# jingjing12110/X-GGM

Measured on AMD Instinct MI355X. Metric: train samples/sec (36-obj VQA batch); one step = plain + GGM pass, each fwd+bwd+clip+BertAdam, higher is better.
Workload: dtype bf16; 1 GPU; 1xMI355X bf16: VQA-CP-v2-shaped synthetic batch=32/GPU, 36 objects x 2048, 20 tokens, A=2274, LXMERT 9/5/5 + GCNx2, full fwd+bwd+clip+BertAdam x2 passes (plain pass first, KL x 8), dropout on, delta=5 branch mix; global_batch=32, parallelism=dp1, order=vqa, world_size=1, zero1=False, hip_graph=True

## Files before the change

### include/xggm.h

```cpp
#ifndef XGGM_H
#define XGGM_H

#include <stddef.h>
#include <stdint.h>

#ifdef __cplusplus
extern "C" {
#endif

typedef struct ihipStream_t* xggm_stream_t;

#define XGGM_VERSION 100

#define XGGM_ACT_NONE 0
#define XGGM_ACT_GELU 1
#define XGGM_ACT_SIGMOID 2
#define XGGM_ACT_TANH 3
#define XGGM_ACT_GELU_GRAD 4

#define XGGM_AGG_PLAIN 0
#define XGGM_AGG_TRANSPOSE 1
#define XGGM_AGG_SYMMETRIZE 2

int xggm_version(void);
// ... 18 lines not shown
    int64_t a_bs, b_bs, c_bs;
    const float* bias;
    const void* residual;
    void* preact;
    const void* aux;
    float* colsum;
    int act, c_f32, accumulate;
    float alpha;
    float* sqsum;
    const float* scale_a;
    const float* scale_b;
    void* c8;
    const float* c8_qscale;
    float* c8_amax;
    int amax_slots;
} xggm_gemm_problem;
int xggm_gemm_grouped_f32(const xggm_gemm_problem* probs, int n, int tile, xggm_stream_t stream);
int xggm_gemm_grouped_bf16(const xggm_gemm_problem* probs, int n, int tile, xggm_stream_t stream);
int xggm_gemm_fp8e4m3(const void* A, const void* B, void* C, int M, int N, int K, int64_t a_rs, int64_t b_ns, int64_t ldc,
                      const float* scale_a, const float* scale_b, const float* bias, const void* residual, void* preact,
                      int act, int c_f32, xggm_stream_t stream);
int xggm_gemm_grouped_fp8e4m3(const xggm_gemm_problem* probs, int n, int tile, xggm_stream_t stream);
int xggm_fp8_scale_update(float* amax, float* hist, float* qscale, float* dscale, int64_t* pos, int n, int hist_len,
                          float margin, int shrink, int bump, int amax_slots, xggm_stream_t stream);
int xggm_quantize_fp8e4m3_f32(const void* x, void* y, int64_t n, const float* qscale, float* amax, xggm_stream_t stream);
int xggm_quantize_fp8e4m3_bf16(const void* x, void* y, int64_t n, const float* qscale, float* amax, xggm_stream_t stream);
int xggm_gemm_set_group_tile(int v);
int xggm_gemm_set_generic(int on);
int xggm_gemm_set_tile(int variant);
int xggm_colsum_f32(const void* x, float* out, int M, int N, int64_t ld, float* ws, size_t ws_bytes,
                    xggm_stream_t stream);
// ... 482 lines not shown
```

### x-ggm_amd/csrc/gemm.hip

```cpp
#include "common.h"
#include "xggm.h"

namespace {

typedef __attribute__((ext_vector_type(8))) short short8_t;
typedef __attribute__((ext_vector_type(4))) float float4_t;

struct GemmArgs {
    const void* A = nullptr;
    const void* B = nullptr;
    void* C = nullptr;
    int M = 0, N = 0, K = 0;
    int64_t a_rs = 0, a_ks = 0, b_ns = 0, b_ks = 0, ldc = 0;
    int64_t a_bs = 0, b_bs = 0, c_bs = 0;
    const float* bias = nullptr;
    const void* residual = nullptr;
    void* preact = nullptr;
    const void* aux = nullptr;
    float* colsum = nullptr;
    float* sqsum = nullptr;
    unsigned char* c8 = nullptr;
    const float* c8_qscale = nullptr;
    float* c8_amax = nullptr;
    int amax_slots = 1;
    const float* scale_a = nullptr;
    const float* scale_b = nullptr;
    int act = 0;
    int c_f32 = 0;
    int accumulate = 0;
    float alpha = 1.f;
    int a_mode = 0, b_mode = 0;
    int a_tail = 0, b_tail = 0;
    int a_rows = 0, b_rows = 0;
    int xcd_swizzle = 1;
    int batch = 1;
    int use_glds = 1;
    struct TileMap {
        int gx, gy, gxy;
        int xr, xc, rh, rw;
// ... 433 lines not shown
                    {
                        const float4 a = *reinterpret_cast<const float4*>(sp);
                        const float4 c4 = *reinterpret_cast<const float4*>(sp + 4);
                        v[0] = a.x; v[1] = a.y; v[2] = a.z; v[3] = a.w; v[4] = c4.x; v[5] = c4.y; v[6] = c4.z; v[7] = c4.w;
                    }
#pragma unroll
                    for (int e = 0; e < 8; ++e) v[e] = g.alpha * v[e] + bias[e];
                    if (pre) {
                        short8_t pv;
#pragma unroll
                        for (int e = 0; e < 8; ++e) {
                            const bf16 t = __float2bfloat16(v[e]);
                            pv[e] = __builtin_bit_cast(short, t);
                            v[e] = __bfloat162float(t);
                        }
                        *reinterpret_cast<short8_t*>(pre + idx[b]) = pv;
                    }
                    if (g.act == XGGM_ACT_GELU) {
#pragma unroll
                        for (int e = 0; e < 8; ++e) v[e] = gelu_f(v[e]);
                    } else if (g.act == XGGM_ACT_GELU_GRAD) {
#pragma unroll
                        for (int e = 0; e < 8; ++e)
                            v[e] *= gelu_grad_f(__bfloat162float(__builtin_bit_cast(bf16, (short)raux[b][e])));
                    } else if (g.act != XGGM_ACT_NONE) {
#pragma unroll 1
                        for (int e = 0; e < 8; ++e) v[e] = act_apply<bf16>(g.act, v[e], 0.f);
                    }
                    if (res) {
#pragma unroll
                        for (int e = 0; e < 8; ++e) v[e] += __bfloat162float(__builtin_bit_cast(bf16, (short)rres[b][e]));
                    }
                    if (g.colsum) {
                        *reinterpret_cast<float4*>(sp) = make_float4(v[0], v[1], v[2], v[3]);
                        *reinterpret_cast<float4*>(sp + 4) = make_float4(v[4], v[5], v[6], v[7]);
                    }
                    if (g.c8) {
#pragma unroll
                        for (int e = 0; e < 8; ++e) amax8 = fmaxf(amax8, fabsf(v[e]));
                        *reinterpret_cast<int2*>(g.c8 + idx[b]) =
                            make_int2(pack4_e4m3(v[0], v[1], v[2], v[3], q8), pack4_e4m3(v[4], v[5], v[6], v[7], q8));
                    }
                    if (g.c_f32) {
                        float* c = reinterpret_cast<float*>(g.C) + idx[b];
                        float4 o0 = make_float4(v[0], v[1], v[2], v[3]), o1 = make_float4(v[4], v[5], v[6], v[7]);
                        if (g.accumulate) {
                            o0.x += p0[b].x; o0.y += p0[b].y; o0.z += p0[b].z; o0.w += p0[b].w;
                            o1.x += p1[b].x; o1.y += p1[b].y; o1.z += p1[b].z; o1.w += p1[b].w;
                        }
                        if (g.sqsum)
                            sq_add(h * HALF + lr0 + (it0 + b) * RPI, (o0.x * o0.x + o0.y * o0.y) + (o0.z * o0.z + o0.w * o0.w) +
                                                                         (o1.x * o1.x + o1.y * o1.y) + (o1.z * o1.z + o1.w * o1.w));
                        typedef float __attribute__((ext_vector_type(4))) f4;
                        __builtin_nontemporal_store((f4){o0.x, o0.y, o0.z, o0.w}, reinterpret_cast<f4*>(c));
                        __builtin_nontemporal_store((f4){o1.x, o1.y, o1.z, o1.w}, reinterpret_cast<f4*>(c + 4));
                    } else {
                        if (g.accumulate) {
#pragma unroll
                            for (int e = 0; e < 8; ++e) v[e] += __bfloat162float(__builtin_bit_cast(bf16, (short)rprev[b][e]));
                        }
                        short8_t ov;
#pragma unroll
                        for (int e = 0; e < 8; ++e) ov[e] = __builtin_bit_cast(short, __float2bfloat16(v[e]));
                        *reinterpret_cast<short8_t*>(reinterpret_cast<bf16*>(g.C) + idx[b]) = ov;
                    }
                }
            }
        } else {
#pragma unroll 1
            for (int it = 0; it < ITER; ++it) {
                const int lr = lr0 + it * RPI, row = m0 + h * HALF + lr;
                if (row >= g.M || !col_ok) continue;
                const int nval = min(8, g.N - col);
                const int64_t idx = coff + (int64_t)row * g.ldc + col;
#pragma unroll 1
                for (int e = 0; e < nval; ++e) {
                    float x = g.alpha * stage[lr * LDS_LD + lc + e] + (g.bias ? g.bias[col + e] : 0.f);
                    if (pre) {
                        pre[idx + e] = __float2bfloat16(x);
// ... 95 lines not shown
#pragma unroll
    for (int j = 0; j < TN; ++j)
        bias[j] = (g.bias && col0 + j * 16 < g.N) ? *reinterpret_cast<const float4_t*>(g.bias + col0 + j * 16)
                                                  : (float4_t){0.f, 0.f, 0.f, 0.f};
    const Q8 qs(KIND == 1 && g.c8 ? g.c8_qscale : nullptr);
    const float q8 = qs.q, alpha = g.alpha;
    float amax8 = 0.f, sq = 0.f;
#ifdef XGGM_STAMP
    if (g.ablate & 0x10000) asm volatile("s_waitcnt vmcnt(0)" ::: "memory");
#endif
    TRACE(g, 1);
    const int off0 = row0 * g.ldc + col0;
    float* cf = reinterpret_cast<float*>(g.C) + coff;
    bf16* cb = reinterpret_cast<bf16*>(g.C) + coff;
    bf16* pre = reinterpret_cast<bf16*>(g.preact) + coff;
#pragma unroll
    for (int i = 0; i < TM; ++i) {
        if (i == 1) STAMP(g, 3);
        TRACE(g, 2 + i);
        if (row0 + i * 16 >= g.M) continue;
#pragma unroll
        for (int j = 0; j < TN; ++j) {
            if (col0 + j * 16 >= g.N) continue;
            const int off = off0 + i * 16 * g.ldc + j * 16;
            float4_t v = alpha * acc[i][j] + bias[j];
            if (KIND == 1) {
                short4v pv;
#pragma unroll
                for (int e = 0; e < 4; ++e) {
                    const bf16 t = __float2bfloat16(v[e]);
                    pv[e] = __builtin_bit_cast(short, t);
                    v[e] = gelu_f(__bfloat162float(t));
                }
                *reinterpret_cast<short4v*>(pre + off) = pv;
                if (g.c8) {
                    amax8 = fmaxf(fmaxf(amax8, fmaxf(fabsf(v[0]), fabsf(v[1]))), fmaxf(fabsf(v[2]), fabsf(v[3])));
                    *reinterpret_cast<int*>(g.c8 + coff + off) = pack4_e4m3(v[0], v[1], v[2], v[3], q8);
                }
            }
            if (KIND == 0 && g.c_f32) {
                sq += (v[0] * v[0] + v[1] * v[1]) + (v[2] * v[2] + v[3] * v[3]);
                __builtin_nontemporal_store(v, reinterpret_cast<float4_t*>(cf + off));
            } else {
                short4v ov;
#pragma unroll
                for (int e = 0; e < 4; ++e) ov[e] = __builtin_bit_cast(short, __float2bfloat16(v[e]));
                if (!ABLATE(g, 4) || ov[0] == 12345) *reinterpret_cast<short4v*>(cb + off) = ov;
            }
        }
    }
    if (KIND == 1 && g.c8 && g.c8_amax) {
        const float wv = wave_max(amax8);
        if (lane == 0) stage[wid] = wv;
        lds_barrier();
        if (tid == 0) {
            float bm = stage[0];
#pragma unroll
            for (int w = 1; w < W; ++w) bm = fmaxf(bm, stage[w]);
            if (bm > qs.thr) amax_record(g.c8_amax, g.amax_slots, (int)(blockIdx.x + blockIdx.y * gridDim.x), bm);
        }
    }
    if (KIND == 0 && g.sqsum) {
// ... 789 lines not shown
            *rows = (R + VEC - 1) / VEC * VEC;
            return 2;
        }
    }
    return 0;
}

GemmArgs from_problem(const xggm_gemm_problem& p, const GemmHooks& h) {
    GemmArgs g;
    g.A = p.A; g.B = p.B; g.C = p.C; g.M = p.M; g.N = p.N; g.K = p.K;
    g.a_rs = p.a_rs; g.a_ks = p.a_ks; g.b_ns = p.b_ns; g.b_ks = p.b_ks; g.ldc = p.ldc;
    g.a_bs = p.a_bs; g.b_bs = p.b_bs; g.c_bs = p.c_bs;
    g.bias = p.bias; g.residual = p.residual; g.preact = p.preact; g.aux = p.aux; g.colsum = p.colsum; g.sqsum = p.sqsum;
    g.c8 = reinterpret_cast<unsigned char*>(p.c8); g.c8_qscale = p.c8_qscale; g.c8_amax = p.c8_amax;
    g.amax_slots = p.amax_slots > 1 ? p.amax_slots : 1;
    g.scale_a = p.scale_a; g.scale_b = p.scale_b;
    g.act = p.act; g.c_f32 = p.c_f32; g.accumulate = p.accumulate; g.alpha = p.alpha;
    g.xcd_swizzle = h.xcd_swizzle; g.batch = p.batch; g.use_glds = h.glds; SET_STAMP(g);
    return g;
}

template <typename T> int launch(GemmArgs g, int batch, const GemmHooks& h, hipStream_t stream) {
    XGGM_REQUIRE(g.M > 0 && g.N > 0 && g.K > 0 && batch > 0, "xggm_gemm: empty problem M=%d N=%d K=%d batch=%d", g.M, g.N,
                 g.K, batch);
    XGGM_REQUIRE(g.A && g.B && g.C, "xggm_gemm: null operand");
    XGGM_REQUIRE(g.act >= 0 && g.act <= XGGM_ACT_GELU_GRAD, "xggm_gemm: bad activation %d", g.act);
    XGGM_REQUIRE(g.act != XGGM_ACT_GELU_GRAD || g.aux, "xggm_gemm: GELU_GRAD needs aux");
    XGGM_REQUIRE(g.ldc >= g.N, "xggm_gemm: ldc %lld < N %d", (long long)g.ldc, g.N);
    XGGM_REQUIRE(!g.sqsum || g.c_f32, "xggm_gemm: sqsum is defined for fp32 outputs");
    g.a_mode = pick_mode<T>(g.A, g.a_rs, g.a_ks, g.a_bs, g.M, g.K, &g.a_tail, &g.a_rows);
// ... 109 lines not shown
                nkmax = std::max(nkmax, nk);
            }
            const float r = std::max(1.0, tiles / 256.0);
            const float est = std::max(tm.a + tm.b * r + tm.s * (float)(work / 256.0), tm.f + tm.k * nkmax);
            if (v == 0 || est < best) {
                best = est;
                v = c + 1;
            }
        }
    }
    return v;
}

inline bool group_tile_ok(int tile) { return (tile >= 0 && tile <= 4) || (tile >= 7 && tile <= 9); }

template <typename T> int grouped(const xggm_gemm_problem* probs, int n, int tile, const GemmHooks h, hipStream_t stream) {
    XGGM_REQUIRE(probs && n > 0, "xggm_gemm_grouped: no problems");
    XGGM_REQUIRE(group_tile_ok(tile), "xggm_gemm_grouped: tile %d (0: the library chooses; 1-4, 7-9: see xggm.h)", tile);
    const int pin = tile ? tile : h.group_tile;
    bool fast = sizeof(T) == 2 && !h.force_generic && n <= MAX_GROUP;
    GroupArgs ga;
    ga.nprob = n;
    for (int i = 0; i < n && fast; ++i) {
        GemmArgs g = from_problem(probs[i], h);
        if (!(g.M > 0 && g.N > 0 && g.K > 0 && g.batch > 0 && g.A && g.B && g.C)) fast = false;
        g.a_mode = pick_mode<T>(g.A, g.a_rs, g.a_ks, g.a_bs, g.M, g.K, &g.a_tail, &g.a_rows);
        g.b_mode = pick_mode<T>(g.B, g.b_ns, g.b_ks, g.b_bs, g.N, g.K, &g.b_tail, &g.b_rows);
        if (g.a_mode == 0 || g.b_mode == 0) fast = false;
        ga.p[i] = g;
    }
    for (int i = 1; i < n && fast; ++i)
        for (int j = i; j > 0 && ga.p[j].K > ga.p[j - 1].K; --j) std::swap(ga.p[j], ga.p[j - 1]);
    if (!fast || (n == 1 && !(h.single_grouped && glds_ok<false>(ga.p[0])))) {
// ... 24 lines not shown
        if (ok)
            return v == 7 ? launch_grouped_role<128, 128>(ga, stream)
                          : v == 8 ? launch_grouped_role<128, 64>(ga, stream) : launch_grouped_role<64, 64>(ga, stream);
        v = v == 7 ? 3 : v == 8 ? 2 : 1;
    }
    if (v == 4) return launch_grouped_tile<128, 128, 8>(ga, h, stream);
    if (v == 3) return launch_grouped_tile<128, 128>(ga, h, stream);
    if (v == 2) return launch_grouped_tile<128, 64>(ga, h, stream);
    return launch_grouped_tile<64, 64>(ga, h, stream);
}
}

extern "C" int xggm_gemm_grouped_fp8e4m3(const xggm_gemm_problem* probs, int n, int tile, hipStream_t stream) {
    XGGM_REQUIRE(probs && n > 0 && n <= MAX_GROUP, "xggm_gemm_grouped_fp8e4m3: 1..%d problems per launch (n = %d)", MAX_GROUP, n);
    XGGM_REQUIRE(group_tile_ok(tile), "xggm_gemm_grouped_fp8e4m3: tile %d (0: the library chooses; 1-4, 7-9: see xggm.h)", tile);
    const GemmHooks h = g_hooks;
    const int pin = tile ? tile : h.group_tile;
    GroupArgs ga;
    ga.nprob = n;
    for (int i = 0; i < n; ++i) {
        GemmArgs g = from_problem(probs[i], h);
        XGGM_REQUIRE(g.M > 0 && g.N > 0 && g.K > 0 && g.batch > 0 && g.A && g.B && g.C,
                     "xggm_gemm_grouped_fp8e4m3: empty problem or null operand (%d)", i);
        XGGM_REQUIRE(g.a_ks == 1 && g.b_ks == 1, "xggm_gemm_grouped_fp8e4m3: e4m3 operands are k-contiguous");
        XGGM_REQUIRE(g.K % 16 == 0 && g.a_rs % 16 == 0 && g.b_ns % 16 == 0 && g.a_rs >= g.K && g.b_ns >= g.K &&
                         g.a_bs % 16 == 0 && g.b_bs % 16 == 0,
                     "xggm_gemm_grouped_fp8e4m3: K, row and batch strides must be multiples of 16 (K = %d)", g.K);
        XGGM_REQUIRE(reinterpret_cast<uintptr_t>(g.A) % 16 == 0 && reinterpret_cast<uintptr_t>(g.B) % 16 == 0,
                     "xggm_gemm_grouped_fp8e4m3: operands must be 16-byte aligned");
        XGGM_REQUIRE(g.act >= 0 && g.act < XGGM_ACT_GELU_GRAD && !g.aux && !g.colsum && !g.sqsum && !g.accumulate,
// ... 63 lines not shown
```

### x-ggm_amd/functional.py

```python
import os

import torch
from torch.autograd import Function

from . import ops

F32 = torch.float32


class ScalarSlot:
    __slots__ = ("t",)

    def __init__(self, t):
        self.t = t


class Runtime:

    def __init__(self, arena, seed=9595):
        self.arena = arena
        self.rng = ops.make_rng(seed, arena.device)
        ops.sum_ws(arena.device)
        self.training = True
        self.p_hidden = 0.1
# ... 220 lines not shown
    H = xq.shape[1]
    heads = att.num_attention_heads
    wq, wk, wv = att.query.weight, att.key.weight, att.value.weight
    bq, bk, bv = att.query.bias, att.key.bias, att.value.bias
    self_att = xkv is None
    f8 = a.fp8 if xq.dtype == torch.bfloat16 else None
    emit, use8 = f8 is not None, f8 is not None and f8.active

    if emit:
        xq8, sq = f8.get(xq, ("in", id(att), salt, 0))
        if not self_att:
            xkv8, skv = f8.get(xkv, ("in", id(att), salt, 1))
    if self_att:
        if use8:
            w8, sw = f8.w8([wq, wk, wv])
            p1, qkv, _ = ops.p_fwd8(xq8, w8, sq, sw, a.fused([bq, bk, bv]))
            p1.is8 = True
        else:
            p1, qkv, _ = ops.p_fwd(xq, a.fused([wq, wk, wv]), a.fused([bq, bk, bv]))
        kv = None
        yield [p1]
        q, k, v = qkv[:, :H], qkv[:, H:2 * H], qkv[:, 2 * H:]
    else:
        if use8:
            w8q, sw = f8.w8(wq)
            w8kv, _ = f8.w8([wk, wv])
            p1, qkv, _ = ops.p_fwd8(xq8, w8q, sq, sw, bq.data)
            p2, kv, _ = ops.p_fwd8(xkv8, w8kv, skv, sw, a.fused([bk, bv]))
            p1.is8 = p2.is8 = True
        else:
            p1, qkv, _ = ops.p_fwd(xq, a.w(wq), bq.data)
            p2, kv, _ = ops.p_fwd(xkv, a.fused([wk, wv]), a.fused([bk, bv]))
        yield [p1, p2]
        q, k, v = qkv, kv[:, :H], kv[:, H:]
    p_att, p_hid = rt.p(rt.p_attn), rt.p(rt.p_hidden)
    e_ctx = f8.emit(("ctx", id(att), salt)) if emit else (None, None)
    core = ops.AttnFwdReq(q, k, v, mask, B, heads, Sq, Sk, p_att, rt.rng, att._sid + salt, emit8=e_ctx[0])
    core.prefetch = (a.after(wv, 9 * H * H, use8),)
    yield core
    c = core.out
    if use8 and core.out8 is not None:
        w8o, swo = f8.w8(outm.dense.weight)
        p3, h, _ = ops.p_fwd8(core.out8, w8o, f8.dscale[e_ctx[1]:e_ctx[1] + 1], swo, None)
        p3.is8 = True
    else:
        p3, h, _ = ops.p_fwd(c, a.w(outm.dense.weight), None)
    yield [p3]
    e_ln = f8.emit(("ln", id(outm), salt)) if emit else (None, None)
    ln = ops.LnFwdReq(h, outm.dense.bias.data, xq, outm.LayerNorm.weight.data, outm.LayerNorm.bias.data, 1e-12,
                      p_pre=p_hid, rng=rt.rng, sid_pre=outm._sid + salt, emit8=e_ln[0])
    ln.prefetch = (a.after(outm.dense.weight, 3 * H * H // 2, use8, skip=8 * H * H),)
    yield ln
    if emit:
        f8.put(ln.out, ln.out8, e_ln[1])
    return ln.out, (att, outm, (B, Sq, Sk, heads, H, p_att, p_hid, self_att, salt),
                    (xq, xkv, mask, qkv, kv, c, ln.z, ln.stats))


def g_attn_bwd(rt, saved, dy, defer_wgrad=False, link=None):
    att, outm, dims, tens = saved
    B, Sq, Sk, heads, H, p_att, p_hid, self_att, salt = dims
    xq, xkv, mask, qkv, kv, c, z, stats = tens
    a = rt.arena
    wq, wk, wv = att.query.weight, att.key.weight, att.value.weight
    bq, bk, bv = att.query.bias, att.key.bias, att.value.bias
    lb = ops.LnBwdReq(dy.contiguous(), z, stats, outm.LayerNorm.weight.data, a.atomic_target(outm.LayerNorm.weight),
                      a.atomic_target(outm.LayerNorm.bias), a.atomic_target(outm.dense.bias), p_pre=p_hid, rng=rt.rng,
                      sid_pre=outm._sid + salt, defer=rt.defer_list())
    if a.shadow is not None:
        lb.prefetch = (a.w(outm.dense.weight).view(-1),)
    yield lb
    d_h, d_res = lb.d_in, lb.d_res
    pd, d_c = ops.p_dgrad(d_h, a.w(outm.dense.weight))
    if defer_wgrad:
        yield [pd]
        late = [_p_wgrad(rt, d_h, c, outm.dense.weight)]
    else:
        yield [_p_wgrad(rt, d_h, c, outm.dense.weight), pd]
        late = []
    if self_att:
        dqkv = torch.empty_like(qkv)
        gb = a.atomic_target([bq, bk, bv])
        ab = ops.AttnBwdReq(qkv[:, :H], qkv[:, H:2 * H], qkv[:, 2 * H:], mask, d_c, dqkv[:, :H], dqkv[:, H:2 * H],
                            dqkv[:, 2 * H:], B, heads, Sq, Sk, p_att, rt.rng, att._sid + salt, gb[:H], gb[H:2 * H],
                            gb[2 * H:], defer=rt.defer_list())
        if a.shadow is not None:
            ab.prefetch = (a.fused([wq, wk, wv]).view(-1), a.before(wq, 8 * H * H))
        yield ab
        pdx, dxq = ops.p_dgrad(dqkv, a.fused([wq, wk, wv]), residual=d_res)
        dxkv = None
        if defer_wgrad:
            yield late + [pdx]
            yield [_p_wgrad(rt, dqkv, xq, [wq, wk, wv])]
        else:
            yield [_p_wgrad(rt, dqkv, xq, [wq, wk, wv]), pdx]
    else:
        dq = torch.empty_like(qkv)
        dkv = torch.empty_like(kv)
        gbq, gbkv = a.atomic_target(bq), a.atomic_target([bk, bv])
        yield ops.AttnBwdReq(qkv, kv[:, :H], kv[:, H:], mask, d_c, dq, dkv[:, :H], dkv[:, H:], B, heads, Sq, Sk, p_att,
                             rt.rng, att._sid + salt, gbq, gbkv[:H], gbkv[H:], defer=rt.defer_list())
        if defer_wgrad and link is not None and "dxq" in link:
            yield late
            pdq, dxq = ops.p_dgrad(dq, a.w(wq), residual=d_res, into=link["dxkv"])
            pdk, dxkv = ops.p_dgrad(dkv, a.fused([wk, wv]), into=link["dxq"])
            yield [_p_wgrad(rt, dq, xq, wq), _p_wgrad(rt, dkv, xkv, [wk, wv]), pdq, pdk]
            return dxq, dxkv
        pdq, dxq = ops.p_dgrad(dq, a.w(wq), residual=d_res)
        pdk, dxkv = ops.p_dgrad(dkv, a.fused([wk, wv]))
        if link is not None:
            link["dxq"], link["dxkv"] = dxq, dxkv
        if defer_wgrad:
            yield late + [pdq, pdk]
            yield [_p_wgrad(rt, dq, xq, wq), _p_wgrad(rt, dkv, xkv, [wk, wv])]
        else:
            yield [_p_wgrad(rt, dq, xq, wq), _p_wgrad(rt, dkv, xkv, [wk, wv]), pdq, pdk]
    return dxq, dxkv


_SPLIT_K = int(os.environ.get("XGGM_SPLIT_K", "2"))


def g_ffn_fwd(rt, inter, outm, x):
    a = rt.arena
    f8 = a.fp8 if x.dtype == torch.bfloat16 else None
    emit, use8 = f8 is not None, f8 is not None and f8.active
    act8 = e_act = None
    if emit:
        x8, sx = f8.get(x, ("in", id(inter), 0, 0))
        e_act = f8.emit(("act", id(inter)))
        act8 = torch.empty((x.shape[0], inter.dense.weight.shape[0]), device=x.device, dtype=torch.uint8)
        e8 = (act8,) + e_act[0]
    if use8:
        w8, sw = f8.w8(inter.dense.weight)
        p1, act, u = ops.p_fwd8(x8, w8, sx, sw, inter.dense.bias.data, act=ops.ACT_GELU, want_preact=True, emit8=e8)
        p1.is8 = True
    else:
        p1, act, u = ops.p_fwd(x, a.w(inter.dense.weight), inter.dense.bias.data, act=ops.ACT_GELU, want_preact=True,
                               emit8=e8 if emit else None)
    yield [p1]
    w2 = a.w(outm.dense.weight)
    S = _SPLIT_K if (x.dtype == torch.bfloat16 and w2.shape[1] >= 2048 and w2.shape[1] % (128 * max(_SPLIT_K, 1)) == 0) else 0
    if use8:
        w8, sw = f8.w8(outm.dense.weight)
        p2, h, _ = ops.p_fwd8(act8, w8, f8.dscale[e_act[1]:e_act[1] + 1], sw, None, split=S if S > 1 else 0)
        p2.is8 = True
    elif S > 1:
        p2, h = ops.p_fwd_splitk(act, w2, S)
    else:
        p2, h, _ = ops.p_fwd(act, w2, None)
    yield [p2]
    p_hid = rt.p(rt.p_hidden)
    e_ln = f8.emit(("ln", id(outm), 0)) if emit else (None, None)
    ln = ops.LnFwdReq(h, outm.dense.bias.data, x, outm.LayerNorm.weight.data, outm.LayerNorm.bias.data, 1e-12,
                      p_pre=p_hid, rng=rt.rng, sid_pre=outm._sid, dtype=x.dtype, emit8=e_ln[0])
    ln.prefetch = (a.after(outm.dense.weight, 3 * x.shape[1] * x.shape[1] // 2, use8, skip=3 * x.shape[1] * x.shape[1] // 2),)
    yield ln
    if emit:
        f8.put(ln.out, ln.out8, e_ln[1])
    return ln.out, (inter, outm, p_hid, (x, u, act, ln.z, ln.stats))


def g_ffn_bwd(rt, saved, dy):
    inter, outm, p_hid, (x, u, act, z, stats) = saved
    a = rt.arena
    lb = ops.LnBwdReq(dy.contiguous(), z, stats, outm.LayerNorm.weight.data, a.atomic_target(outm.LayerNorm.weight),
                      a.atomic_target(outm.LayerNorm.bias), a.atomic_target(outm.dense.bias), p_pre=p_hid, rng=rt.rng,
                      sid_pre=outm._sid, defer=rt.defer_list())
    yield lb
    d_h, d_res = lb.d_in, lb.d_res
    pd, d_u = ops.p_dgrad(d_h, a.w(outm.dense.weight), gelu_aux=u, colsum=a.atomic_target(inter.dense.bias),
                          defer=rt.defer_list())
    yield [_p_wgrad(rt, d_h, act, outm.dense.weight), pd]
    pdx, dx = ops.p_dgrad(d_u, a.w(inter.dense.weight), residual=d_res)
    yield [_p_wgrad(rt, d_u, x, inter.dense.weight), pdx]
    return dx


class AttnBlockFn(Function):

    @staticmethod
    def forward(ctx, rt, att, outm, xq, xkv, mask, B, Sq, Sk, salt, *params):
        ctx.np = len(params)
        (res,) = drive(xq.dtype, [g_attn_fwd(rt, att, outm, xq, xkv, mask, B, Sq, Sk, salt)])
        y, ctx.saved = res
        ctx.rt = rt
        return y

    @staticmethod
# ... 575 lines not shown
```

### x-ggm_amd/ops.py

```python
import torch

from . import _lib
from ._lib import call, ptr, stream

ACT_NONE, ACT_GELU, ACT_SIGMOID, ACT_TANH, ACT_GELU_GRAD = 0, 1, 2, 3, 4
AGG_PLAIN, AGG_TRANSPOSE, AGG_SYMMETRIZE = 0, 1, 2
F32 = torch.float32
BF16 = torch.bfloat16


def sfx(dt):
    if dt == F32:
        return "f32"
    if dt == BF16:
        return "bf16"
    raise TypeError("xggm_amd supports float32 and bfloat16 activations, got %s" % dt)


def _chk(t, dt=None, name="tensor"):
    if not t.is_cuda:
        raise RuntimeError("xggm_amd: %s must live on the GPU (no CPU fallback)" % name)
    if dt is not None and t.dtype != dt:
        raise TypeError("xggm_amd: %s has dtype %s, expected %s" % (name, t.dtype, dt))
    return t
# ... 106 lines not shown

import ctypes as _ct
import os


class GemmProblem(_ct.Structure):
    _fields_ = [("A", _ct.c_void_p), ("B", _ct.c_void_p), ("C", _ct.c_void_p),
                ("M", _ct.c_int), ("N", _ct.c_int), ("K", _ct.c_int),
                ("a_rs", _ct.c_int64), ("a_ks", _ct.c_int64), ("b_ns", _ct.c_int64), ("b_ks", _ct.c_int64),
                ("ldc", _ct.c_int64), ("batch", _ct.c_int),
                ("a_bs", _ct.c_int64), ("b_bs", _ct.c_int64), ("c_bs", _ct.c_int64),
                ("bias", _ct.c_void_p), ("residual", _ct.c_void_p), ("preact", _ct.c_void_p), ("aux", _ct.c_void_p),
                ("colsum", _ct.c_void_p), ("act", _ct.c_int), ("c_f32", _ct.c_int), ("accumulate", _ct.c_int), ("alpha", _ct.c_float),
                ("sqsum", _ct.c_void_p),
                ("scale_a", _ct.c_void_p), ("scale_b", _ct.c_void_p), ("c8", _ct.c_void_p), ("c8_qscale", _ct.c_void_p),
                ("c8_amax", _ct.c_void_p), ("amax_slots", _ct.c_int)]


def _problem(A, B, C, M, N, K, a_rs, a_ks, b_ns, b_ks, ldc, bias=None, residual=None, preact=None, aux=None,
             act=ACT_NONE, c_f32=False, accumulate=False, colsum=None):
    p = GemmProblem(ptr(A), ptr(B), ptr(C), M, N, K, a_rs, a_ks, b_ns, b_ks, ldc, 1, 0, 0, 0, ptr(bias),
                    ptr(residual), ptr(preact), ptr(aux), ptr(colsum), act, int(c_f32), int(accumulate), 1.0)
    p.keep = (A, B, C, bias, residual, preact, aux, colsum)
    return p


def p_fwd(x, w, bias=None, act=ACT_NONE, want_preact=False, out_f32=False, emit8=None):
    M, K, a_rs = _rows(_chk(x))
    N = w.shape[0]
    assert w.shape[1] == K and w.dtype == x.dtype and w.is_contiguous()
    y = torch.empty((M, N), device=x.device, dtype=F32 if out_f32 else x.dtype)
    pre = torch.empty((M, N), device=x.device, dtype=x.dtype) if want_preact else None
    p = _problem(x, w, y, M, N, K, a_rs, 1, K, 1, N, bias=bias, preact=pre, act=act, c_f32=out_f32)
    if emit8 is not None:
        y8, q, amax = emit8
        assert y8.shape == y.shape and y8.element_size() == 1 and y8.is_contiguous() and x.dtype == BF16 and not out_f32
        p.c8, p.c8_qscale, p.c8_amax = ptr(y8), ptr(q), ptr(amax)
        p.amax_slots = amax.numel() if amax is not None else 0
        p.keep = p.keep + (y8, q, amax)
    return p, y, pre


def p_fwd_splitk(x, w, S):
    M, K, a_rs = _rows(_chk(x))
    N = w.shape[0]
    assert w.shape[1] == K and w.dtype == x.dtype and w.is_contiguous()
    if K % (64 * S):
        raise RuntimeError("p_fwd_splitk: K = %d is not a multiple of 64 * %d" % (K, S))
    part = torch.empty((S, M, N), device=x.device, dtype=F32)
    p = _problem(x, w, part, M, N, K // S, a_rs, 1, K, 1, N, c_f32=True)
    p.batch, p.a_bs, p.b_bs, p.c_bs = S, K // S, K // S, M * N
    return p, part


def p_fwd8(x8, w8, sx, sw, bias=None, act=ACT_NONE, want_preact=False, emit8=None, split=0):
    M, K, a_rs = _rows(_chk(x8))
    N = w8.shape[0]
    assert w8.shape[1] == K and x8.element_size() == 1 and w8.element_size() == 1 and w8.stride(1) == 1
    if split > 1:
        if K % (128 * split):
            raise RuntimeError("p_fwd8: K = %d is not a multiple of 128 * %d" % (K, split))
        y = torch.empty((split, M, N), device=x8.device, dtype=F32)
        p = _problem(x8, w8, y, M, N, K // split, a_rs, 1, w8.stride(0), 1, N, c_f32=True)
        p.batch, p.a_bs, p.b_bs, p.c_bs = split, K // split, K // split, M * N
        pre = None
    else:
        y = torch.empty((M, N), device=x8.device, dtype=BF16)
        pre = torch.empty((M, N), device=x8.device, dtype=BF16) if want_preact else None
        p = _problem(x8, w8, y, M, N, K, a_rs, 1, w8.stride(0), 1, N, bias=bias, preact=pre, act=act)
    p.scale_a, p.scale_b = ptr(sx), ptr(sw)
    p.keep = p.keep + (sx, sw)
    if emit8 is not None:
        y8, q, amax = emit8
        assert y8.shape == y.shape and y8.element_size() == 1 and y8.is_contiguous()
        p.c8, p.c8_qscale, p.c8_amax = ptr(y8), ptr(q), ptr(amax)
        p.amax_slots = amax.numel() if amax is not None else 0
        p.keep = p.keep + (y8, q, amax)
    return p, y, pre


GROUP_MAX = 6


def gemm_group8(problems, tile=0):
    gemm_group("e4m3", problems, tile)


def p_dgrad(dy, w, residual=None, gelu_aux=None, colsum=None, into=None, defer=None):
    M, N, a_rs = _rows(_chk(dy))
    K = w.shape[1]
    assert w.shape[0] == N and w.dtype == dy.dtype and w.is_contiguous()
    if into is not None:
        assert tuple(into.shape) == (M, K) and into.dtype == dy.dtype and into.is_contiguous()
        assert gelu_aux is None and colsum is None
        return _problem(dy, w, into, M, K, N, a_rs, 1, 1, K, K, residual=residual, accumulate=True), into
    dx = torch.empty((M, K), device=dy.device, dtype=dy.dtype)
    part = job = None
    if colsum is not None:
        _c(colsum, F32, "colsum")
        assert colsum.numel() == K
        if K % 4:
            raise RuntimeError("p_dgrad: column sums need a width that is a multiple of 4 (got %d)" % K)
        part = torch.empty((colsum_rows(M), K), device=dy.device, dtype=F32)
        job = (part, colsum_rows(M), 1, K, (colsum,))
    p = _problem(dy, w, dx, M, K, N, a_rs, 1, 1, K, K, residual=residual, aux=gelu_aux,
                 act=ACT_GELU_GRAD if gelu_aux is not None else ACT_NONE, colsum=part)
    if job is not None:
        if defer is not None:
            defer.append(job)
        else:
            p.post = job
    return p, dx


def p_wgrad(dy, x, gw, accumulate, sqsum=None):
    M, N, dy_rs = _rows(_chk(dy))
    M2, K, x_rs = _rows(_chk(x))
    assert M2 == M and x.dtype == dy.dtype and tuple(gw.shape) == (N, K) and gw.is_contiguous()
    assert gw.dtype == F32 or gw.dtype == dy.dtype
    p = _problem(dy, x, gw, N, K, M, 1, dy_rs, 1, x_rs, K, c_f32=gw.dtype == F32, accumulate=accumulate)
    if sqsum is not None:
# ... 1535 lines not shown
```

Measured before the change: 2991 samples/s.

## Add per-site GEMM store cache policies and a wide permlane-paired bf16 epilogue

Adds a store-policy field to the GEMM problem (plain, nontemporal, or write-through with sc1) that is chosen per call site (qkv, ffn1, dgrad use write-through by default), so outputs consumed soon by the next kernel can stay in or bypass cache as suits them. It also rewrites the small-tile bf16 epilogue to pair adjacent 16x16 blocks with permlane16_swap, so each lane issues 16-byte stores instead of 8-byte ones when the address is aligned. Inline asm stores and the new lane swaps add risk around correctness and alignment edge cases, and write-through may add memory traffic.

New measurement: 2960 samples/s. 0.99x the previous value.

```diff
diff --git a/include/xggm.h b/include/xggm.h
--- a/include/xggm.h
+++ b/include/xggm.h
@@ -56,7 +56,10 @@
     const float* c8_qscale;
     float* c8_amax;
     int amax_slots;
+    int store;
 } xggm_gemm_problem;
+enum { XGGM_STORE_DEFAULT = 0, XGGM_STORE_PLAIN = 1, XGGM_STORE_NT = 2, XGGM_STORE_WT = 3, XGGM_STORE_NARROW = 0x10,
+       XGGM_STORE_PREACT_SHIFT = 8 };
 int xggm_gemm_grouped_f32(const xggm_gemm_problem* probs, int n, int tile, xggm_stream_t stream);
 int xggm_gemm_grouped_bf16(const xggm_gemm_problem* probs, int n, int tile, xggm_stream_t stream);
 int xggm_gemm_fp8e4m3(const void* A, const void* B, void* C, int M, int N, int K, int64_t a_rs, int64_t b_ns, int64_t ldc,
diff --git a/x-ggm_amd/csrc/gemm.hip b/x-ggm_amd/csrc/gemm.hip
--- a/x-ggm_amd/csrc/gemm.hip
+++ b/x-ggm_amd/csrc/gemm.hip
@@ -5,6 +5,22 @@
 
 typedef __attribute__((ext_vector_type(8))) short short8_t;
 typedef __attribute__((ext_vector_type(4))) float float4_t;
+
+enum { ST_PLAIN = 1, ST_NT = 2, ST_WT = 3, ST_NARROW = 16 };
+typedef unsigned uint2v __attribute__((ext_vector_type(2)));
+typedef unsigned uint4v __attribute__((ext_vector_type(4)));
+template <typename V> __device__ __forceinline__ void store16(void* p, const V& v, int pol) {
+    static_assert(sizeof(V) == 16, "store16");
+    if (pol == ST_WT)
+        asm volatile("global_store_dwordx4 %0, %1, off sc1\n\ts_nop 1" ::"v"(p), "v"(__builtin_bit_cast(uint4v, v)) : "memory");
+    else if (pol == ST_NT) __builtin_nontemporal_store(v, reinterpret_cast<V*>(p));
+    else *reinterpret_cast<V*>(p) = v;
+}
+template <typename V> __device__ __forceinline__ void store_narrow(void* p, const V& v, int pol) {
+    static_assert(sizeof(V) <= 8, "store_narrow");
+    if (pol == ST_NT) __builtin_nontemporal_store(v, reinterpret_cast<V*>(p));
+    else *reinterpret_cast<V*>(p) = v;
+}
 
 struct GemmArgs {
     const void* A = nullptr;
@@ -23,6 +39,7 @@
     const float* c8_qscale = nullptr;
     float* c8_amax = nullptr;
     int amax_slots = 1;
+    int store = ST_PLAIN | ST_PLAIN << 2;
     const float* scale_a = nullptr;
     const float* scale_b = nullptr;
     int act = 0;
@@ -486,7 +503,7 @@
                             pv[e] = __builtin_bit_cast(short, t);
                             v[e] = __bfloat162float(t);
                         }
-                        *reinterpret_cast<short8_t*>(pre + idx[b]) = pv;
+                        store16(pre + idx[b], pv, (g.store >> 2) & 3);
                     }
                     if (g.act == XGGM_ACT_GELU) {
 #pragma unroll
@@ -510,8 +527,8 @@
                     if (g.c8) {
 #pragma unroll
                         for (int e = 0; e < 8; ++e) amax8 = fmaxf(amax8, fabsf(v[e]));
-                        *reinterpret_cast<int2*>(g.c8 + idx[b]) =
-                            make_int2(pack4_e4m3(v[0], v[1], v[2], v[3], q8), pack4_e4m3(v[4], v[5], v[6], v[7], q8));
+                        store_narrow(g.c8 + idx[b], (uint2v){(unsigned)pack4_e4m3(v[0], v[1], v[2], v[3], q8),
+                                                             (unsigned)pack4_e4m3(v[4], v[5], v[6], v[7], q8)}, g.store & 3);
                     }
                     if (g.c_f32) {
                         float* c = reinterpret_cast<float*>(g.C) + idx[b];
@@ -523,9 +540,8 @@
                         if (g.sqsum)
                             sq_add(h * HALF + lr0 + (it0 + b) * RPI, (o0.x * o0.x + o0.y * o0.y) + (o0.z * o0.z + o0.w * o0.w) +
                                                                          (o1.x * o1.x + o1.y * o1.y) + (o1.z * o1.z + o1.w * o1.w));
-                        typedef float __attribute__((ext_vector_type(4))) f4;
-                        __builtin_nontemporal_store((f4){o0.x, o0.y, o0.z, o0.w}, reinterpret_cast<f4*>(c));
-                        __builtin_nontemporal_store((f4){o1.x, o1.y, o1.z, o1.w}, reinterpret_cast<f4*>(c + 4));
+                        store16(c, (float4_t){o0.x, o0.y, o0.z, o0.w}, g.store & 3);
+                        store16(c + 4, (float4_t){o1.x, o1.y, o1.z, o1.w}, g.store & 3);
                     } else {
                         if (g.accumulate) {
 #pragma unroll
@@ -534,7 +550,7 @@
                         short8_t ov;
 #pragma unroll
                         for (int e = 0; e < 8; ++e) ov[e] = __builtin_bit_cast(short, __float2bfloat16(v[e]));
-                        *reinterpret_cast<short8_t*>(reinterpret_cast<bf16*>(g.C) + idx[b]) = ov;
+                        store16(reinterpret_cast<bf16*>(g.C) + idx[b], ov, g.store & 3);
                     }
                 }
             }
@@ -660,38 +676,113 @@
     float* cf = reinterpret_cast<float*>(g.C) + coff;
     bf16* cb = reinterpret_cast<bf16*>(g.C) + coff;
     bf16* pre = reinterpret_cast<bf16*>(g.preact) + coff;
-#pragma unroll
-    for (int i = 0; i < TM; ++i) {
-        if (i == 1) STAMP(g, 3);
-        TRACE(g, 2 + i);
-        if (row0 + i * 16 >= g.M) continue;
-#pragma unroll
-        for (int j = 0; j < TN; ++j) {
-            if (col0 + j * 16 >= g.N) continue;
-            const int off = off0 + i * 16 * g.ldc + j * 16;
-            float4_t v = alpha * acc[i][j] + bias[j];
-            if (KIND == 1) {
-                short4v pv;
-#pragma unroll
-                for (int e = 0; e < 4; ++e) {
-                    const bf16 t = __float2bfloat16(v[e]);
-                    pv[e] = __builtin_bit_cast(short, t);
-                    v[e] = gelu_f(__bfloat162float(t));
+    const int pol = g.store & 3, pol_pre = (g.store >> 2) & 3;
+    auto pack_bf16 = [](const float4_t& v) {
+        short4v o;
+#pragma unroll
+        for (int e = 0; e < 4; ++e) o[e] = __builtin_bit_cast(short, __float2bfloat16(v[e]));
+        return __builtin_bit_cast(uint2v, o);
+    };
+    if ((KIND == 0 && g.c_f32) || (g.store & ST_NARROW)) {
+#pragma unroll
+        for (int i = 0; i < TM; ++i) {
+            if (i == 1) STAMP(g, 3);
+            TRACE(g, 2 + i);
+            if (row0 + i * 16 >= g.M) continue;
+#pragma unroll
+            for (int j = 0; j < TN; ++j) {
+                if (col0 + j * 16 >= g.N) continue;
+                const int off = off0 + i * 16 * g.ldc + j * 16;
+                float4_t v = alpha * acc[i][j] + bias[j];
+                if (KIND == 1) {
+                    short4v pv;
+#pragma unroll
+                    for (int e = 0; e < 4; ++e) {
+                        const bf16 t = __float2bfloat16(v[e]);
+                        pv[e] = __builtin_bit_cast(short, t);
+                        v[e] = gelu_f(__bfloat162float(t));
+                    }
+                    store_narrow(pre + off, pv, pol_pre);
+                    if (g.c8) {
+                        amax8 = fmaxf(fmaxf(amax8, fmaxf(fabsf(v[0]), fabsf(v[1]))), fmaxf(fabsf(v[2]), fabsf(v[3])));
+                        store_narrow(g.c8 + coff + off, pack4_e4m3(v[0], v[1], v[2], v[3], q8), pol);
+                    }
                 }
-                *reinterpret_cast<short4v*>(pre + off) = pv;
-                if (g.c8) {
-                    amax8 = fmaxf(fmaxf(amax8, fmaxf(fabsf(v[0]), fabsf(v[1]))), fmaxf(fabsf(v[2]), fabsf(v[3])));
-                    *reinterpret_cast<int*>(g.c8 + coff + off) = pack4_e4m3(v[0], v[1], v[2], v[3], q8);
+                if (KIND == 0 && g.c_f32) {
+                    sq += (v[0] * v[0] + v[1] * v[1]) + (v[2] * v[2] + v[3] * v[3]);
+                    store16(cf + off, v, pol);
+                } else {
+                    const uint2v ov = pack_bf16(v);
+                    if (!ABLATE(g, 4) || ov[0] == 12345) store_narrow(cb + off, ov, pol);
                 }
             }
-            if (KIND == 0 && g.c_f32) {
-                sq += (v[0] * v[0] + v[1] * v[1]) + (v[2] * v[2] + v[3] * v[3]);
-                __builtin_nontemporal_store(v, reinterpret_cast<float4_t*>(cf + off));
+        }
+    } else {
+        static_assert(TN % 2 == 0, "the wide epilogue pairs 16 x 16 blocks along N");
+        int wl = lane;
+        asm volatile("" : "+v"(wl));
+        const int wq = wl >> 4;
+        const int wcol0 = n0 + wn + (wq & 1) * 16 + (wq >> 1) * 8;
+        const int woff0 = (m0 + wm + (wl & 15)) * g.ldc + wcol0;
+        const bool c16 = reinterpret_cast<uintptr_t>(cb + woff0) % 16 == 0;
+        const bool p16 = KIND == 1 && reinterpret_cast<uintptr_t>(pre + woff0) % 16 == 0;
+        const bool q8al = KIND == 1 && reinterpret_cast<uintptr_t>(g.c8 + coff + woff0) % 8 == 0;
+        auto swap = [](unsigned& lo, unsigned& hi) {
+            const auto r = __builtin_amdgcn_permlane16_swap(lo, hi, false, false);
+            lo = r[0];
+            hi = r[1];
+        };
+        auto put = [&](bf16* dst, uint2v lo, uint2v hi, bool al16, int ncol, int sp) {
+            unsigned l0 = lo[0], l1 = lo[1], h0 = hi[0], h1 = hi[1];
+            swap(l0, h0);
+            swap(l1, h1);
+            if (ncol < 4) return;
+            if (ncol >= 8 && al16) {
+                store16(dst, (uint4v){l0, l1, h0, h1}, sp);
             } else {
-                short4v ov;
-#pragma unroll
-                for (int e = 0; e < 4; ++e) ov[e] = __builtin_bit_cast(short, __float2bfloat16(v[e]));
-                if (!ABLATE(g, 4) || ov[0] == 12345) *reinterpret_cast<short4v*>(cb + off) = ov;
+                store_narrow(dst, (uint2v){l0, l1}, sp);
+                if (ncol >= 8) store_narrow(dst + 4, (uint2v){h0, h1}, sp);
+            }
+        };
+#pragma unroll
+        for (int i = 0; i < TM; ++i) {
+            if (i == 1) STAMP(g, 3);
+            TRACE(g, 2 + i);
+            if (row0 + i * 16 >= g.M) continue;
+#pragma unroll
+            for (int j = 0; j < TN; j += 2) {
+                if (n0 + wn + j * 16 >= g.N) continue;
+                const int off = woff0 + i * 16 * g.ldc + j * 16;
+                const int ncol = g.N - (wcol0 + j * 16);
+                float4_t va = alpha * acc[i][j] + bias[j], vb = alpha * acc[i][j + 1] + bias[j + 1];
+                if (KIND == 1) {
+                    short4v pa, pb;
+#pragma unroll
+                    for (int e = 0; e < 4; ++e) {
+                        const bf16 ta = __float2bfloat16(va[e]), tb = __float2bfloat16(vb[e]);
+                        pa[e] = __builtin_bit_cast(short, ta);
+                        pb[e] = __builtin_bit_cast(short, tb);
+                        va[e] = gelu_f(__bfloat162float(ta));
+                        vb[e] = gelu_f(__bfloat162float(tb));
+                    }
+                    put(pre + off, __builtin_bit_cast(uint2v, pa), __builtin_bit_cast(uint2v, pb), p16, ncol, pol_pre);
+                    if (g.c8) {
+                        if (col0 + j * 16 < g.N)
+                            amax8 = fmaxf(fmaxf(amax8, fmaxf(fabsf(va[0]), fabsf(va[1]))), fmaxf(fabsf(va[2]), fabsf(va[3])));
+                        if (col0 + j * 16 + 16 < g.N)
+                            amax8 = fmaxf(fmaxf(amax8, fmaxf(fabsf(vb[0]), fabsf(vb[1]))), fmaxf(fabsf(vb[2]), fabsf(vb[3])));
+                        unsigned lo = pack4_e4m3(va[0], va[1], va[2], va[3], q8), hi = pack4_e4m3(vb[0], vb[1], vb[2], vb[3], q8);
+                        swap(lo, hi);
+                        unsigned char* q = g.c8 + coff + off;
+                        if (ncol >= 8 && q8al) {
+                            store_narrow(q, (uint2v){lo, hi}, pol);
+                        } else {
+                            if (ncol >= 4) store_narrow(q, lo, pol);
+                            if (ncol >= 8) store_narrow(q + 4, hi, pol);
+                        }
+                    }
+                }
+                put(cb + off, pack_bf16(va), pack_bf16(vb), c16, (!ABLATE(g, 4) || va[0] == 12345.f) ? ncol : 0, pol);
             }
         }
     }
@@ -1511,6 +1602,11 @@
     g.bias = p.bias; g.residual = p.residual; g.preact = p.preact; g.aux = p.aux; g.colsum = p.colsum; g.sqsum = p.sqsum;
     g.c8 = reinterpret_cast<unsigned char*>(p.c8); g.c8_qscale = p.c8_qscale; g.c8_amax = p.c8_amax;
     g.amax_slots = p.amax_slots > 1 ? p.amax_slots : 1;
+    {
+        const int c = p.store & 3, pre = (p.store >> XGGM_STORE_PREACT_SHIFT) & 3;
+        const int rc = c ? c : (p.c_f32 ? ST_NT : ST_PLAIN);
+        g.store = rc | (pre ? pre : rc) << 2 | ((p.store & XGGM_STORE_NARROW) ? ST_NARROW : 0);
+    }
     g.scale_a = p.scale_a; g.scale_b = p.scale_b;
     g.act = p.act; g.c_f32 = p.c_f32; g.accumulate = p.accumulate; g.alpha = p.alpha;
     g.xcd_swizzle = h.xcd_swizzle; g.batch = p.batch; g.use_glds = h.glds; SET_STAMP(g);
@@ -1650,9 +1746,20 @@
 
 inline bool group_tile_ok(int tile) { return (tile >= 0 && tile <= 4) || (tile >= 7 && tile <= 9); }
 
+static_assert(sizeof(xggm_gemm_problem) == 224 && offsetof(xggm_gemm_problem, store) == 220,
+              "xggm_gemm_problem.store lies in the former tail padding: the size of the struct is part of the ABI");
+inline int bad_store(const xggm_gemm_problem* probs, int n) {
+    for (int i = 0; i < n; ++i)
+        if (probs[i].store & ~(3 | XGGM_STORE_NARROW | 3 << XGGM_STORE_PREACT_SHIFT)) return i;
+    return -1;
+}
+
 template <typename T> int grouped(const xggm_gemm_problem* probs, int n, int tile, const GemmHooks h, hipStream_t stream) {
     XGGM_REQUIRE(probs && n > 0, "xggm_gemm_grouped: no problems");
     XGGM_REQUIRE(group_tile_ok(tile), "xggm_gemm_grouped: tile %d (0: the library chooses; 1-4, 7-9: see xggm.h)", tile);
+    const int bs = probs && n > 0 ? bad_store(probs, n) : -1;
+    XGGM_REQUIRE(bs < 0, "xggm_gemm_grouped: store %d of problem %d (policy 0-3, | 0x10 narrow, | policy << 8 for preact: see xggm.h)",
+                 probs[bs < 0 ? 0 : bs].store, bs);
     const int pin = tile ? tile : h.group_tile;
     bool fast = sizeof(T) == 2 && !h.force_generic && n <= MAX_GROUP;
     GroupArgs ga;
@@ -1707,6 +1814,9 @@
 extern "C" int xggm_gemm_grouped_fp8e4m3(const xggm_gemm_problem* probs, int n, int tile, hipStream_t stream) {
     XGGM_REQUIRE(probs && n > 0 && n <= MAX_GROUP, "xggm_gemm_grouped_fp8e4m3: 1..%d problems per launch (n = %d)", MAX_GROUP, n);
     XGGM_REQUIRE(group_tile_ok(tile), "xggm_gemm_grouped_fp8e4m3: tile %d (0: the library chooses; 1-4, 7-9: see xggm.h)", tile);
+    const int bs = bad_store(probs, n);
+    XGGM_REQUIRE(bs < 0, "xggm_gemm_grouped_fp8e4m3: store %d of problem %d (policy 0-3, | 0x10 narrow, | policy << 8 for preact: see xggm.h)",
+                 probs[bs < 0 ? 0 : bs].store, bs);
     const GemmHooks h = g_hooks;
     const int pin = tile ? tile : h.group_tile;
     GroupArgs ga;
diff --git a/x-ggm_amd/functional.py b/x-ggm_amd/functional.py
--- a/x-ggm_amd/functional.py
+++ b/x-ggm_amd/functional.py
@@ -258,10 +258,10 @@
     if self_att:
         if use8:
             w8, sw = f8.w8([wq, wk, wv])
-            p1, qkv, _ = ops.p_fwd8(xq8, w8, sq, sw, a.fused([bq, bk, bv]))
+            p1, qkv, _ = ops.p_fwd8(xq8, w8, sq, sw, a.fused([bq, bk, bv]), site="qkv")
             p1.is8 = True
         else:
-            p1, qkv, _ = ops.p_fwd(xq, a.fused([wq, wk, wv]), a.fused([bq, bk, bv]))
+            p1, qkv, _ = ops.p_fwd(xq, a.fused([wq, wk, wv]), a.fused([bq, bk, bv]), site="qkv")
         kv = None
         yield [p1]
         q, k, v = qkv[:, :H], qkv[:, H:2 * H], qkv[:, 2 * H:]
@@ -269,12 +269,12 @@
         if use8:
             w8q, sw = f8.w8(wq)
             w8kv, _ = f8.w8([wk, wv])
-            p1, qkv, _ = ops.p_fwd8(xq8, w8q, sq, sw, bq.data)
-            p2, kv, _ = ops.p_fwd8(xkv8, w8kv, skv, sw, a.fused([bk, bv]))
+            p1, qkv, _ = ops.p_fwd8(xq8, w8q, sq, sw, bq.data, site="qkv")
+            p2, kv, _ = ops.p_fwd8(xkv8, w8kv, skv, sw, a.fused([bk, bv]), site="qkv")
             p1.is8 = p2.is8 = True
         else:
-            p1, qkv, _ = ops.p_fwd(xq, a.w(wq), bq.data)
-            p2, kv, _ = ops.p_fwd(xkv, a.fused([wk, wv]), a.fused([bk, bv]))
+            p1, qkv, _ = ops.p_fwd(xq, a.w(wq), bq.data, site="qkv")
+            p2, kv, _ = ops.p_fwd(xkv, a.fused([wk, wv]), a.fused([bk, bv]), site="qkv")
         yield [p1, p2]
         q, k, v = qkv, kv[:, :H], kv[:, H:]
     p_att, p_hid = rt.p(rt.p_attn), rt.p(rt.p_hidden)
@@ -285,10 +285,10 @@
     c = core.out
     if use8 and core.out8 is not None:
         w8o, swo = f8.w8(outm.dense.weight)
-        p3, h, _ = ops.p_fwd8(core.out8, w8o, f8.dscale[e_ctx[1]:e_ctx[1] + 1], swo, None)
+        p3, h, _ = ops.p_fwd8(core.out8, w8o, f8.dscale[e_ctx[1]:e_ctx[1] + 1], swo, None, site="attn_out")
         p3.is8 = True
     else:
-        p3, h, _ = ops.p_fwd(c, a.w(outm.dense.weight), None)
+        p3, h, _ = ops.p_fwd(c, a.w(outm.dense.weight), None, site="attn_out")
     yield [p3]
     e_ln = f8.emit(("ln", id(outm), salt)) if emit else (None, None)
     ln = ops.LnFwdReq(h, outm.dense.bias.data, xq, outm.LayerNorm.weight.data, outm.LayerNorm.bias.data, 1e-12,
@@ -315,7 +315,7 @@
         lb.prefetch = (a.w(outm.dense.weight).view(-1),)
     yield lb
     d_h, d_res = lb.d_in, lb.d_res
-    pd, d_c = ops.p_dgrad(d_h, a.w(outm.dense.weight))
+    pd, d_c = ops.p_dgrad(d_h, a.w(outm.dense.weight), site="dgrad")
     if defer_wgrad:
         yield [pd]
         late = [_p_wgrad(rt, d_h, c, outm.dense.weight)]
@@ -331,7 +331,7 @@
         if a.shadow is not None:
             ab.prefetch = (a.fused([wq, wk, wv]).view(-1), a.before(wq, 8 * H * H))
         yield ab
-        pdx, dxq = ops.p_dgrad(dqkv, a.fused([wq, wk, wv]), residual=d_res)
+        pdx, dxq = ops.p_dgrad(dqkv, a.fused([wq, wk, wv]), residual=d_res, site="dgrad")
         dxkv = None
         if defer_wgrad:
             yield late + [pdx]
@@ -346,12 +346,12 @@
                              rt.rng, att._sid + salt, gbq, gbkv[:H], gbkv[H:], defer=rt.defer_list())
         if defer_wgrad and link is not None and "dxq" in link:
             yield late
-            pdq, dxq = ops.p_dgrad(dq, a.w(wq), residual=d_res, into=link["dxkv"])
-            pdk, dxkv = ops.p_dgrad(dkv, a.fused([wk, wv]), into=link["dxq"])
+            pdq, dxq = ops.p_dgrad(dq, a.w(wq), residual=d_res, into=link["dxkv"], site="dgrad")
+            pdk, dxkv = ops.p_dgrad(dkv, a.fused([wk, wv]), into=link["dxq"], site="dgrad")
             yield [_p_wgrad(rt, dq, xq, wq), _p_wgrad(rt, dkv, xkv, [wk, wv]), pdq, pdk]
             return dxq, dxkv
-        pdq, dxq = ops.p_dgrad(dq, a.w(wq), residual=d_res)
-        pdk, dxkv = ops.p_dgrad(dkv, a.fused([wk, wv]))
+        pdq, dxq = ops.p_dgrad(dq, a.w(wq), residual=d_res, site="dgrad")
+        pdk, dxkv = ops.p_dgrad(dkv, a.fused([wk, wv]), site="dgrad")
         if link is not None:
             link["dxq"], link["dxkv"] = dxq, dxkv
         if defer_wgrad:
@@ -377,22 +377,22 @@
         e8 = (act8,) + e_act[0]
     if use8:
         w8, sw = f8.w8(inter.dense.weight)
-        p1, act, u = ops.p_fwd8(x8, w8, sx, sw, inter.dense.bias.data, act=ops.ACT_GELU, want_preact=True, emit8=e8)
+        p1, act, u = ops.p_fwd8(x8, w8, sx, sw, inter.dense.bias.data, act=ops.ACT_GELU, want_preact=True, emit8=e8, site="ffn1")
         p1.is8 = True
     else:
         p1, act, u = ops.p_fwd(x, a.w(inter.dense.weight), inter.dense.bias.data, act=ops.ACT_GELU, want_preact=True,
-                               emit8=e8 if emit else None)
+                               emit8=e8 if emit else None, site="ffn1")
     yield [p1]
     w2 = a.w(outm.dense.weight)
     S = _SPLIT_K if (x.dtype == torch.bfloat16 and w2.shape[1] >= 2048 and w2.shape[1] % (128 * max(_SPLIT_K, 1)) == 0) else 0
     if use8:
         w8, sw = f8.w8(outm.dense.weight)
-        p2, h, _ = ops.p_fwd8(act8, w8, f8.dscale[e_act[1]:e_act[1] + 1], sw, None, split=S if S > 1 else 0)
+        p2, h, _ = ops.p_fwd8(act8, w8, f8.dscale[e_act[1]:e_act[1] + 1], sw, None, split=S if S > 1 else 0, site="ffn2")
         p2.is8 = True
     elif S > 1:
-        p2, h = ops.p_fwd_splitk(act, w2, S)
+        p2, h = ops.p_fwd_splitk(act, w2, S, site="ffn2")
     else:
-        p2, h, _ = ops.p_fwd(act, w2, None)
+        p2, h, _ = ops.p_fwd(act, w2, None, site="ffn2")
     yield [p2]
     p_hid = rt.p(rt.p_hidden)
     e_ln = f8.emit(("ln", id(outm), 0)) if emit else (None, None)
@@ -414,9 +414,9 @@
     yield lb
     d_h, d_res = lb.d_in, lb.d_res
     pd, d_u = ops.p_dgrad(d_h, a.w(outm.dense.weight), gelu_aux=u, colsum=a.atomic_target(inter.dense.bias),
-                          defer=rt.defer_list())
+                          defer=rt.defer_list(), site="dgrad")
     yield [_p_wgrad(rt, d_h, act, outm.dense.weight), pd]
-    pdx, dx = ops.p_dgrad(d_u, a.w(inter.dense.weight), residual=d_res)
+    pdx, dx = ops.p_dgrad(d_u, a.w(inter.dense.weight), residual=d_res, site="dgrad")
     yield [_p_wgrad(rt, d_u, x, inter.dense.weight), pdx]
     return dx
 
diff --git a/x-ggm_amd/ops.py b/x-ggm_amd/ops.py
--- a/x-ggm_amd/ops.py
+++ b/x-ggm_amd/ops.py
@@ -144,24 +144,64 @@
                 ("colsum", _ct.c_void_p), ("act", _ct.c_int), ("c_f32", _ct.c_int), ("accumulate", _ct.c_int), ("alpha", _ct.c_float),
                 ("sqsum", _ct.c_void_p),
                 ("scale_a", _ct.c_void_p), ("scale_b", _ct.c_void_p), ("c8", _ct.c_void_p), ("c8_qscale", _ct.c_void_p),
-                ("c8_amax", _ct.c_void_p), ("amax_slots", _ct.c_int)]
+                ("c8_amax", _ct.c_void_p), ("amax_slots", _ct.c_int), ("store", _ct.c_int)]
+
+
+STORE_DEFAULT, STORE_PLAIN, STORE_NT, STORE_WT, STORE_NARROW, STORE_PREACT_SHIFT = 0, 1, 2, 3, 0x10, 8
+STORE_SITES = {
+    "qkv": STORE_WT,
+    "attn_out": STORE_DEFAULT,
+    "ffn1": STORE_WT,
+    "ffn1_pre": STORE_DEFAULT,
+    "ffn2": STORE_DEFAULT,
+    "dgrad": STORE_WT,
+}
+
+
+def _store_hook():
+    spec = os.environ.get("XGGM_STORE")
+    if not spec:
+        return
+    for item in spec.split(","):
+        site, _, val = item.partition("=")
+        v = int(val, 0)
+        if site == "all":
+            for k in STORE_SITES:
+                STORE_SITES[k] = v
+        elif site in STORE_SITES:
+            STORE_SITES[site] = v
+        else:
+            raise RuntimeError("XGGM_STORE: unknown site %r (sites: %s)" % (site, ", ".join(STORE_SITES)))
+
+
+_store_hook()
+
+
+def site_store(site):
+    if site is None:
+        return STORE_DEFAULT
+    v = STORE_SITES[site]
+    if site == "ffn1":
+        v |= (STORE_SITES["ffn1_pre"] & 3) << STORE_PREACT_SHIFT
+    return v
 
 
 def _problem(A, B, C, M, N, K, a_rs, a_ks, b_ns, b_ks, ldc, bias=None, residual=None, preact=None, aux=None,
-             act=ACT_NONE, c_f32=False, accumulate=False, colsum=None):
+             act=ACT_NONE, c_f32=False, accumulate=False, colsum=None, site=None):
     p = GemmProblem(ptr(A), ptr(B), ptr(C), M, N, K, a_rs, a_ks, b_ns, b_ks, ldc, 1, 0, 0, 0, ptr(bias),
                     ptr(residual), ptr(preact), ptr(aux), ptr(colsum), act, int(c_f32), int(accumulate), 1.0)
+    p.store = site_store(site)
     p.keep = (A, B, C, bias, residual, preact, aux, colsum)
     return p
 
 
-def p_fwd(x, w, bias=None, act=ACT_NONE, want_preact=False, out_f32=False, emit8=None):
+def p_fwd(x, w, bias=None, act=ACT_NONE, want_preact=False, out_f32=False, emit8=None, site=None):
     M, K, a_rs = _rows(_chk(x))
     N = w.shape[0]
     assert w.shape[1] == K and w.dtype == x.dtype and w.is_contiguous()
     y = torch.empty((M, N), device=x.device, dtype=F32 if out_f32 else x.dtype)
     pre = torch.empty((M, N), device=x.device, dtype=x.dtype) if want_preact else None
-    p = _problem(x, w, y, M, N, K, a_rs, 1, K, 1, N, bias=bias, preact=pre, act=act, c_f32=out_f32)
+    p = _problem(x, w, y, M, N, K, a_rs, 1, K, 1, N, bias=bias, preact=pre, act=act, c_f32=out_f32, site=site)
     if emit8 is not None:
         y8, q, amax = emit8
         assert y8.shape == y.shape and y8.element_size() == 1 and y8.is_contiguous() and x.dtype == BF16 and not out_f32
@@ -171,19 +211,19 @@
     return p, y, pre
 
 
-def p_fwd_splitk(x, w, S):
+def p_fwd_splitk(x, w, S, site=None):
     M, K, a_rs = _rows(_chk(x))
     N = w.shape[0]
     assert w.shape[1] == K and w.dtype == x.dtype and w.is_contiguous()
     if K % (64 * S):
         raise RuntimeError("p_fwd_splitk: K = %d is not a multiple of 64 * %d" % (K, S))
     part = torch.empty((S, M, N), device=x.device, dtype=F32)
-    p = _problem(x, w, part, M, N, K // S, a_rs, 1, K, 1, N, c_f32=True)
+    p = _problem(x, w, part, M, N, K // S, a_rs, 1, K, 1, N, c_f32=True, site=site)
     p.batch, p.a_bs, p.b_bs, p.c_bs = S, K // S, K // S, M * N
     return p, part
 
 
-def p_fwd8(x8, w8, sx, sw, bias=None, act=ACT_NONE, want_preact=False, emit8=None, split=0):
+def p_fwd8(x8, w8, sx, sw, bias=None, act=ACT_NONE, want_preact=False, emit8=None, split=0, site=None):
     M, K, a_rs = _rows(_chk(x8))
     N = w8.shape[0]
     assert w8.shape[1] == K and x8.element_size() == 1 and w8.element_size() == 1 and w8.stride(1) == 1
@@ -191,13 +231,13 @@
         if K % (128 * split):
             raise RuntimeError("p_fwd8: K = %d is not a multiple of 128 * %d" % (K, split))
         y = torch.empty((split, M, N), device=x8.device, dtype=F32)
-        p = _problem(x8, w8, y, M, N, K // split, a_rs, 1, w8.stride(0), 1, N, c_f32=True)
+        p = _problem(x8, w8, y, M, N, K // split, a_rs, 1, w8.stride(0), 1, N, c_f32=True, site=site)
         p.batch, p.a_bs, p.b_bs, p.c_bs = split, K // split, K // split, M * N
         pre = None
     else:
         y = torch.empty((M, N), device=x8.device, dtype=BF16)
         pre = torch.empty((M, N), device=x8.device, dtype=BF16) if want_preact else None
-        p = _problem(x8, w8, y, M, N, K, a_rs, 1, w8.stride(0), 1, N, bias=bias, preact=pre, act=act)
+        p = _problem(x8, w8, y, M, N, K, a_rs, 1, w8.stride(0), 1, N, bias=bias, preact=pre, act=act, site=site)
     p.scale_a, p.scale_b = ptr(sx), ptr(sw)
     p.keep = p.keep + (sx, sw)
     if emit8 is not None:
@@ -216,14 +256,14 @@
     gemm_group("e4m3", problems, tile)
 
 
-def p_dgrad(dy, w, residual=None, gelu_aux=None, colsum=None, into=None, defer=None):
+def p_dgrad(dy, w, residual=None, gelu_aux=None, colsum=None, into=None, defer=None, site=None):
     M, N, a_rs = _rows(_chk(dy))
     K = w.shape[1]
     assert w.shape[0] == N and w.dtype == dy.dtype and w.is_contiguous()
     if into is not None:
         assert tuple(into.shape) == (M, K) and into.dtype == dy.dtype and into.is_contiguous()
         assert gelu_aux is None and colsum is None
-        return _problem(dy, w, into, M, K, N, a_rs, 1, 1, K, K, residual=residual, accumulate=True), into
+        return _problem(dy, w, into, M, K, N, a_rs, 1, 1, K, K, residual=residual, accumulate=True, site=site), into
     dx = torch.empty((M, K), device=dy.device, dtype=dy.dtype)
     part = job = None
     if colsum is not None:
@@ -234,7 +274,7 @@
         part = torch.empty((colsum_rows(M), K), device=dy.device, dtype=F32)
         job = (part, colsum_rows(M), 1, K, (colsum,))
     p = _problem(dy, w, dx, M, K, N, a_rs, 1, 1, K, K, residual=residual, aux=gelu_aux,
-                 act=ACT_GELU_GRAD if gelu_aux is not None else ACT_NONE, colsum=part)
+                 act=ACT_GELU_GRAD if gelu_aux is not None else ACT_NONE, colsum=part, site=site)
     if job is not None:
         if defer is not None:
             defer.append(job)
```
